# intel/neural-speed

Measured on NVIDIA H100. Metric: decode tokens/s + prefill tok/s Llama-2-7B Q4_0 @1 GPU; % HBM roofline, higher is better.
Workload: dtype int8xint4->f32 (q8_0 x q4_0)

## Files before the change

### neural_speed_b200/csrc/abi.cu

```cuda
#include <atomic>
#include <cstdarg>
#include <cstring>
#include <mutex>
#include <unordered_map>
#include <vector>

#include "nsb.cuh"
#include "btla_planes.h"

static thread_local char g_err[512] = "";
static std::atomic<unsigned long long> g_launches{0};

void ns_set_error(const char* fmt, ...) {
  va_list ap;
  va_start(ap, fmt);
  vsnprintf(g_err, sizeof(g_err), fmt, ap);
  va_end(ap);
}
[[noreturn]] void ns_fatal(const char* fmt, ...) {
  va_list ap;
  va_start(ap, fmt);
  fprintf(stderr, "Err: ");
  vfprintf(stderr, fmt, ap);
  fprintf(stderr, "\n");
// ... 753 lines not shown
  if (!ids || ids_stride < 1 || id < 0 || id >= ids_stride || n_as < 1 || n_as > 256 || m < 1) {
    ns_set_error("ns_mul_mat_id: invalid ids (stride=%d id=%d n_as=%d m=%d)", ids_stride, id, n_as, m);
    return NS_E_INVALID;
  }
  std::vector<int32_t> host;
  const int32_t* h = ids;
  if (ids_on_device) {
    host.resize((size_t)m * ids_stride);
    NS_CUDA_TRY(cudaMemcpyAsync(host.data(), ids, host.size() * sizeof(int32_t), cudaMemcpyDeviceToHost, st));
    NS_CUDA_TRY(cudaStreamSynchronize(st));
    h = host.data();
  }
  std::vector<int> count((size_t)n_as, 0);
  for (int t = 0; t < m; ++t) {
    const int e = h[(size_t)t * ids_stride + id];
    if (e < 0 || e >= n_as) {
      ns_set_error("ns_mul_mat_id: expert id %d of token %d outside [0, %d)", e, t, n_as);
      return NS_E_INVALID;
    }
    ++count[(size_t)e];
  }
  pl->span.assign((size_t)n_as, {0, 0});
  int at = 0;
  for (int e = 0; e < n_as; ++e) {
    pl->span[(size_t)e] = {at, at};
    at += count[(size_t)e];
  }
  pl->order.assign((size_t)m, 0);
  for (int t = 0; t < m; ++t) pl->order[(size_t)pl->span[(size_t)h[(size_t)t * ids_stride + id]].second++] = t;
  pl->identity = true;
  for (int t = 0; t < m; ++t) pl->identity = pl->identity && pl->order[(size_t)t] == t;
  return NS_OK;
}

extern "C" int ns_moe_plan(const int32_t* ids, int ids_stride, int id, int m, int n_as, int* order, int* span) {
  ExpertPlan pl;
  if (int rc = plan_experts(ids, ids_stride, id, 0, m, n_as, nullptr, &pl)) return rc;
  if (order) memcpy(order, pl.order.data(), (size_t)m * sizeof(int));
  if (span)
    for (int e = 0; e < n_as; ++e) {
      span[2 * e] = pl.span[(size_t)e].first;
      span[2 * e + 1] = pl.span[(size_t)e].second;
    }
  return pl.identity ? 1 : 0;
}

struct ExpertScratch {
  int* order;
  float *xg, *yg;
  void* ws;
};
static int expert_scratch(const ExpertPlan& pl, int m, int k, int n, size_t mm_ws, cudaStream_t st, ExpertScratch* sc) {
  const size_t ob = ns_round_up((size_t)m * 4, 256), xb = ns_round_up((size_t)m * k * 4, 256), yb = ns_round_up((size_t)m * n * 4, 256);
  char* base = (char*)scratch_get(st, ob + xb + yb + mm_ws + 256);
  if (!base) return NS_E_CUDA;
  sc->order = (int*)base;
  sc->xg = (float*)(base + ob);
  sc->yg = (float*)(base + ob + xb);
  sc->ws = base + ob + xb + yb;
  if (!pl.identity) NS_CUDA_TRY(cudaMemcpyAsync(sc->order, pl.order.data(), (size_t)m * 4, cudaMemcpyHostToDevice, st));
  return NS_OK;
}

extern "C" int ns_mul_mat_id(const ns_weight* const* experts, int n_as, const int32_t* ids, int ids_stride, int id, int ids_on_device,
                             const float* act, int lda, float* dst, int ldo, int m, int flags, void* queue) {
  if (int rc = ns_ensure_device()) return rc;
  if (!experts || !act || !dst || n_as < 1 || m < 1) return NS_E_INVALID;
  for (int e = 0; e < n_as; ++e)
    if (!experts[e] || experts[e]->n != experts[0]->n || experts[e]->k != experts[0]->k) {
      ns_set_error("ns_mul_mat_id: expert %d missing or of another shape", e);
      return NS_E_INVALID;
    }
  const int n = experts[0]->n, k = experts[0]->k;
  if (lda < k || ldo < n) return NS_E_INVALID;
  cudaStream_t st = stream_of(queue);
  ExpertPlan pl;
  if (int rc = plan_experts(ids, ids_stride, id, ids_on_device, m, n_as, st, &pl)) return rc;
  ExpertScratch sc;
  if (int rc = expert_scratch(pl, m, k, n, ns_device_workspace_bytes(m, k), st, &sc)) return rc;
  const float* x = act;
  float* y = dst;
  int ldx = lda, ldy = ldo;
  if (!pl.identity) {
    if (int rc = ns_launch_move_rows(true, act, lda, sc.order, sc.xg, k, m, k, st)) return rc;
    x = sc.xg, y = sc.yg, ldx = k, ldy = n;
  }
  for (int e = 0; e < n_as; ++e) {
    const int b = pl.span[(size_t)e].first, c = pl.span[(size_t)e].second - b;
    if (c == 0) continue;
    if (int rc = mul_mat_impl(experts[e], x + (size_t)b * ldx, ldx, y + (size_t)b * ldy, ldy, c, nullptr, nullptr, flags, sc.ws, (void*)st,
                              nullptr, 0.f))
      return rc;
  }
  if (!pl.identity) return ns_launch_move_rows(false, sc.yg, n, sc.order, dst, ldo, m, n, st);
  return NS_OK;
}

extern "C" int ns_ffn_id(const ns_weight* const* gate, const ns_weight* const* down, const ns_weight* const* up, int n_as, int gelu,
                         const int32_t* ids, int ids_stride, int id, int ids_on_device, const float* act, int lda, float* tmp,
                         float* dst, int ldo, int m, void* queue) {
  if (int rc = ns_ensure_device()) return rc;
  if (!gate || !down || !up || !act || !tmp || !dst || n_as < 1 || m < 1) return NS_E_INVALID;
  for (int e = 0; e < n_as; ++e)
    if (!gate[e] || !down[e] || !up[e] || gate[e]->n != gate[0]->n || gate[e]->k != gate[0]->k || down[e]->n != down[0]->n ||
        down[e]->k != gate[0]->n || up[e]->n != gate[0]->n || up[e]->k != gate[0]->k) {
      ns_set_error("ns_ffn_id: expert %d missing or of another shape", e);
      return NS_E_INVALID;
    }
  const int k = gate[0]->k, fmid = gate[0]->n, n = down[0]->n;
  if (lda < k || ldo < n) return NS_E_INVALID;
  cudaStream_t st = stream_of(queue);
  ExpertPlan pl;
  if (int rc = plan_experts(ids, ids_stride, id, ids_on_device, m, n_as, st, &pl)) return rc;
  ExpertScratch sc;
  if (int rc = expert_scratch(pl, m, k, n, ns_device_workspace_bytes(m, k > fmid ? k : fmid), st, &sc)) return rc;
  const float* x = act;
  float* y = dst;
  int ldx = lda, ldy = ldo;
  if (!pl.identity) {
    if (int rc = ns_launch_move_rows(true, act, lda, sc.order, sc.xg, k, m, k, st)) return rc;
    x = sc.xg, y = sc.yg, ldx = k, ldy = n;
  }
  for (int e = 0; e < n_as; ++e) {
    const int b = pl.span[(size_t)e].first, c = pl.span[(size_t)e].second - b;
    if (c == 0) continue;
    if (int rc = ffn_impl(gate[e], down[e], up[e], gelu ? NS_ELT_GELU : NS_ELT_DEFAULT, nullptr, nullptr, 0, x + (size_t)b * ldx, ldx,
                          tmp + (size_t)2 * b * fmid, y + (size_t)b * ldy, ldy, c, sc.ws, (void*)st))
      return rc;
  }
  if (!pl.identity) return ns_launch_move_rows(false, sc.yg, n, sc.order, dst, ldo, m, n, st);
  return NS_OK;
}

extern "C" int ns_prepare_activation(const ns_weight* w, const float* act, int lda, int m, void* workspace, void* queue) {
  if (int rc = ns_ensure_device()) return rc;
  if (!w || !act || !workspace || m < 1 || m > ns_gemv_tile_rows(w) || lda < w->k) {
    ns_set_error("ns_prepare_activation: invalid arguments (m=%d)", m);
    return NS_E_INVALID;
  }
  return ns_launch_act_prep(act, lda, m, w, workspace, stream_of(queue));
}

extern "C" int ns_matmul_prepared(const ns_weight* const* weights, int nw, int mode, const void* workspace, float* dst,
                                  int ldo, int m, const float* bias, int bias_bcast, const float* residual, float* aux,
                                  void* queue) {
  if (int rc = ns_ensure_device()) return rc;
  if (!weights || nw < 1 || nw > 3 || mode < 0 || mode > 2 || !workspace || !dst) {
    ns_set_error("ns_matmul_prepared: invalid arguments");
    return NS_E_INVALID;
  }
  return ns_launch_gemv(weights, nw, mode, workspace, dst, ldo, m, m, bias, bias_bcast, residual, aux, stream_of(queue));
}

struct ns_graph {
  cudaGraph_t graph;
  cudaGraphExec_t exec;
};
extern "C" int ns_graph_begin(void* queue) {
  if (int rc = ns_ensure_device()) return rc;
  NS_CUDA_TRY(cudaStreamBeginCapture(stream_of(queue), cudaStreamCaptureModeThreadLocal));
  return NS_OK;
}
extern "C" ns_graph* ns_graph_end(void* queue) {
  cudaGraph_t g = nullptr;
  if (!ns_cuda_ok(cudaStreamEndCapture(stream_of(queue), &g), "cudaStreamEndCapture") || !g) return nullptr;
  cudaGraphExec_t e = nullptr;
  if (!ns_cuda_ok(cudaGraphInstantiate(&e, g, 0), "cudaGraphInstantiate")) {
    cudaGraphDestroy(g);
    return nullptr;
  }
  ns_graph* r = new ns_graph();
  r->graph = g;
  r->exec = e;
  return r;
}
extern "C" int ns_graph_launch(ns_graph* g, void* queue) {
  if (!g) return NS_E_INVALID;
  NS_CUDA_TRY(cudaGraphLaunch(g->exec, stream_of(queue)));
  return NS_OK;
}
extern "C" void ns_graph_free(ns_graph* g) {
  if (!g) return;
  cudaGraphExecDestroy(g->exec);
  cudaGraphDestroy(g->graph);
  delete g;
}

extern "C" void bestla_init(void) { (void)ns_ensure_device(); }
extern "C" int bestla_set_threads(int nth) { return nth; }
extern "C" void* bestla_get_thread_handle(void) { return nullptr; }
extern "C" void bestla_timer(bool) {}

extern "C" void* bestla_create_device(bool profile) {
  if (ns_ensure_device()) ns_fatal("bestla_create_device: %s", g_err);
  ns_device* d = new ns_device();
  d->dev = g_default.dev;
  d->profile = profile;
  if (cudaStreamCreateWithFlags(&d->stream, cudaStreamNonBlocking) != cudaSuccess) ns_fatal("cudaStreamCreate failed");
  return d;
}
extern "C" void* bestla_get_device_queue(void* device) { return device ? (void*)((ns_device*)device)->stream : nullptr; }
extern "C" void bestla_release_device(void* device) {
  if (!device) return;
  ns_device* d = (ns_device*)device;
  cudaStreamSynchronize(d->stream);
  {
    std::lock_guard<std::mutex> lk(g_mu);
    auto it = g_scratch.find(d->stream);
    if (it != g_scratch.end()) {
      cudaFree(it->second.p);
      g_scratch.erase(it);
    }
  }
  cudaStreamDestroy(d->stream);
  delete d;
}
extern "C" size_t bestla_device_gmem_size(void* device) {
  (void)device;
  if (ns_ensure_device()) return 0;
  size_t fr = 0, tot = 0;
  cudaMemGetInfo(&fr, &tot);
  return tot;
}
extern "C" void* bestla_device_malloc(size_t size, void* queue) {
  (void)queue;
  if (ns_ensure_device()) ns_fatal("bestla_device_malloc: %s", g_err);
  void* p = nullptr;
  if (cudaMalloc(&p, size) != cudaSuccess) return nullptr;
  return p;
}
extern "C" void bestla_device_free(void* ptr, void* queue) {
  if (!ptr) return;
  cudaStreamSynchronize(stream_of(queue));
  cudaFree(ptr);
}
extern "C" void bestla_device_memcpy(void* dstptr, const void* srcptr, size_t size, void* queue) {
  if (ns_ensure_device()) ns_fatal("bestla_device_memcpy: %s", g_err);
  if (cudaMemcpyAsync(dstptr, srcptr, size, cudaMemcpyDefault, stream_of(queue)) != cudaSuccess)
    ns_fatal("bestla_device_memcpy failed: %s", cudaGetErrorString(cudaGetLastError()));
}
extern "C" void bestla_device_memcpy_sync(void* dstptr, const void* srcptr, size_t size, void* queue) {
  bestla_device_memcpy(dstptr, srcptr, size, queue);
  cudaStreamSynchronize(stream_of(queue));
}
extern "C" void bestla_device_sync(void* queue) {
  if (ns_ensure_device()) ns_fatal("bestla_device_sync: %s", g_err);
  if (cudaStreamSynchronize(stream_of(queue)) != cudaSuccess)
    ns_fatal("bestla_device_sync: %s", cudaGetErrorString(cudaGetLastError()));
}
extern "C" size_t bestla_device_storage_size(void) { return sizeof(ns_weight); }
extern "C" size_t ns_device_storage_bytes(const void* hoststor) {
  BlobView v;
  ns_weight w;
  if (!parse_blob(hoststor, &v) || blob_to_weight_meta(v, &w)) return 0;
  return weight_image_bytes(&w, v.shuffle != nullptr);
}
extern "C" void bestla_device_load_storage(void* hoststor, void* devstor, void* deviceptr, void* queue) {
  if (ns_ensure_device()) ns_fatal("bestla_device_load_storage: %s", g_err);
  BlobView v;
  ns_weight* w = (ns_weight*)devstor;
  if (!devstor || !deviceptr || !parse_blob(hoststor, &v) || blob_to_weight_meta(v, w))
    ns_fatal("bestla_device_load_storage: invalid parameters (%s)", g_err);
  w->base = deviceptr;
  w->external = 1;
  w->total_bytes = weight_image_bytes(w, v.shuffle != nullptr);
  weight_carve(w, deviceptr, v.shuffle != nullptr);
  if (cudaMemsetAsync(deviceptr, 0, w->total_bytes, stream_of(queue)) != cudaSuccess) ns_fatal("cudaMemset failed");
  if (blob_upload_repack(v, w, stream_of(queue))) ns_fatal("bestla_device_load_storage: %s", g_err);
}
extern "C" void bestla_device_f32f32_forward(float* activation, void* weiptr, float* output, int m, int n, int k, int lda,
                                             int ldo, void* workspace, void* queue) {
  const ns_weight* w = (const ns_weight*)weiptr;
  if (!w || w->n != n || w->k != k) ns_fatal("invalid parameters");
  (void)lda;
  if (ns_mul_mat(w, activation, k, output, ldo, m, nullptr, nullptr, 0, workspace, queue))
    ns_fatal("bestla_device_f32f32_forward: %s", g_err);
}

struct CacheEntry {
  ns_weight* w;
  size_t tag;
};
static std::unordered_map<const void*, CacheEntry> g_cache;

static size_t blob_tag(const void* blob, size_t nbytes) {
  size_t t = 1469598103934665603ull;
  const unsigned char* p = (const unsigned char*)blob;
  const size_t head = nbytes < 64 ? nbytes : 64;
  for (size_t i = 0; i < head; ++i) t = (t ^ p[i]) * 1099511628211ull;
  if (nbytes > 72) {
    const size_t span = nbytes - 8, steps = 256;
    for (size_t j = 0; j < steps; ++j) {
      const size_t off = 64 + (size_t)((__uint128_t)(span - 64) * j / steps);
      unsigned long long v;
      memcpy(&v, p + off, 8);
      t = (t ^ (size_t)v) * 1099511628211ull;
    }
  }
  return (t ^ nbytes) * 1099511628211ull;
}
static size_t btla_blob_bytes(const void* blob) {
  size_t msize = 0;
  memcpy(&msize, blob, sizeof(size_t));
  return (msize >= 64 && msize <= ((size_t)1 << 40)) ? msize : 64;
}

// ... 315 lines not shown
```

### neural_speed_b200/csrc/gemv_ring_impl.cuh

```cuda
#pragma once
#include "act_quant.cuh"

namespace {

constexpr int kConsumers = 7;
constexpr int kThreads = (kConsumers + 1) * 32;

__device__ __forceinline__ uint32_t smem_u32(const void* p) { return (uint32_t)__cvta_generic_to_shared(p); }
__device__ __forceinline__ void mbar_init(uint32_t bar, int count) {
  asm volatile("mbarrier.init.shared::cta.b64 [%0], %1;" ::"r"(bar), "r"(count) : "memory");
}
__device__ __forceinline__ void mbar_expect_tx(uint32_t bar, uint32_t bytes) {
  asm volatile("mbarrier.arrive.expect_tx.shared::cta.b64 _, [%0], %1;" ::"r"(bar), "r"(bytes) : "memory");
}
__device__ __forceinline__ void mbar_arrive(uint32_t bar) {
  asm volatile("mbarrier.arrive.shared::cta.b64 _, [%0];" ::"r"(bar) : "memory");
}
__device__ __forceinline__ void mbar_wait(uint32_t bar, uint32_t parity) {
  uint32_t ok;
  do {
    asm volatile(
        "{\n"
        ".reg .pred p;\n"
        "mbarrier.try_wait.parity.shared::cta.b64 p, [%1], %2;\n"
        "selp.u32 %0, 1, 0, p;\n"
        "}\n"
        : "=r"(ok)
        : "r"(bar), "r"(parity)
        : "memory");
  } while (!ok);
}
__device__ __forceinline__ void bulk_g2s(uint32_t dst, const void* src, uint32_t bytes, uint32_t bar) {
  asm volatile("cp.async.bulk.shared::cluster.global.mbarrier::complete_tx::bytes [%0], [%1], %2, [%3];" ::"r"(dst), "l"(src),
               "r"(bytes), "r"(bar)
               : "memory");
}
__device__ __forceinline__ uint4 lds128(uint32_t a) {
  uint4 r;
  asm volatile("ld.shared.v4.u32 {%0,%1,%2,%3}, [%4];" : "=r"(r.x), "=r"(r.y), "=r"(r.z), "=r"(r.w) : "r"(a));
  return r;
}
__device__ __forceinline__ uint2 lds64(uint32_t a) {
  uint2 r;
  asm volatile("ld.shared.v2.u32 {%0,%1}, [%2];" : "=r"(r.x), "=r"(r.y) : "r"(a));
  return r;
}
__device__ __forceinline__ uint32_t lds32(uint32_t a) {
  uint32_t r;
  asm volatile("ld.shared.u32 %0, [%1];" : "=r"(r) : "r"(a));
  return r;
}
__device__ __forceinline__ uint32_t lds16(uint32_t a) {
  unsigned short r;
  asm volatile("ld.shared.u16 %0, [%1];" : "=h"(r) : "r"(a));
  return r;
}
__device__ __forceinline__ int lds8s(uint32_t a) {
  int r;
  asm volatile("ld.shared.s8 %0, [%1];" : "=r"(r) : "r"(a));
  return r;
}
template <int STYPE>
__device__ __forceinline__ float lds_scale(uint32_t base, int idx) {
  if (STYPE == NS_S_F32) return __uint_as_float(lds32(base + 4 * idx));
  if (STYPE == NS_S_F16) return __half2float(__ushort_as_half((unsigned short)lds16(base + 2 * idx)));
  return __uint_as_float(lds16(base + 2 * idx) << 16);
}

struct QuantIn {
  const float* in;
  const float* norm_w;
  float eps;
  int lda, k, kpad, group;
  int act_row, meta_off, meta_stride;
};

__device__ __forceinline__ void sts64(uint32_t a, uint32_t x, uint32_t y) {
  asm volatile("st.shared.v2.u32 [%0], {%1,%2};" ::"r"(a), "r"(x), "r"(y) : "memory");
}
__device__ __forceinline__ float4 ldcg4(const float* p) {
  float4 r;
  asm volatile("ld.global.cg.v4.f32 {%0,%1,%2,%3}, [%4];" : "=f"(r.x), "=f"(r.y), "=f"(r.z), "=f"(r.w) : "l"(p));
  return r;
}
__device__ __forceinline__ float ldcg1(const float* p) {
  float r;
  asm volatile("ld.global.cg.f32 %0, [%1];" : "=f"(r) : "l"(p));
  return r;
}
template <int BAR, int NT>
__device__ __forceinline__ void bar_sync() {
  asm volatile("bar.sync %0, %1;" ::"n"(BAR), "n"(NT) : "memory");
}

template <int NT>
__device__ __forceinline__ void prefetch_norm_w(const float* __restrict__ norm_w, int k, int kpad, int tid, float (&gw)[3][8]) {
  const int ngroups8 = kpad >> 3;
#pragma unroll
  for (int it = 0; it < 3; ++it) {
    const int e = it * NT + tid, k0 = e * 8;
    if (e < ngroups8 && k0 + 8 <= k) {
      const float4 w0 = __ldg(reinterpret_cast<const float4*>(norm_w + k0)), w1 = __ldg(reinterpret_cast<const float4*>(norm_w + k0 + 4));
      gw[it][0] = w0.x; gw[it][1] = w0.y; gw[it][2] = w0.z; gw[it][3] = w0.w;
      gw[it][4] = w1.x; gw[it][5] = w1.y; gw[it][6] = w1.z; gw[it][7] = w1.w;
    } else {
#pragma unroll
      for (int i = 0; i < 8; ++i) gw[it][i] = (e < ngroups8 && k0 + i < k) ? __ldg(norm_w + k0 + i) : 0.f;
    }
  }
}

template <int NI, int NT>
__device__ __forceinline__ void load_passes(const float* row, int eb, int tid, int ngroups8, int k, float (&vv)[NI][8]) {
#pragma unroll
  for (int it = 0; it < NI; ++it) {
    const int e = eb + it * NT + tid;
    const int k0 = e * 8;
    if (e < ngroups8 && k0 + 8 <= k) {
      const float4 x0 = ldcg4(row + k0), x1 = ldcg4(row + k0 + 4);
      vv[it][0] = x0.x; vv[it][1] = x0.y; vv[it][2] = x0.z; vv[it][3] = x0.w;
      vv[it][4] = x1.x; vv[it][5] = x1.y; vv[it][6] = x1.z; vv[it][7] = x1.w;
    } else {
#pragma unroll
      for (int i = 0; i < 8; ++i) vv[it][i] = (e < ngroups8 && k0 + i < k) ? ldcg1(row + k0 + i) : 0.f;
    }
  }
}

template <int COMP, int NT, bool NORM>
__device__ __forceinline__ void quantise_to_smem(const QuantIn& P, int M, uint32_t smem_base, float* red, const float (*gw)[8]) {
  constexpr int NI = 3;
  const int tpb = (COMP == NS_COMP_Q8_0 ? 32 : P.group) >> 3;
  const int ngroups8 = P.kpad >> 3;
  const int tid = threadIdx.x;
  const bool single = ngroups8 <= NI * NT;
  const bool norm = NORM && P.norm_w != nullptr;
  for (int m = 0; m < M; ++m) {
    const float* row = P.in + (size_t)m * P.lda;
    const uint32_t img = smem_base + (uint32_t)m * P.act_row;
    const uint32_t meta = smem_base + P.meta_off + 8u * (uint32_t)(m * P.meta_stride);
    float vv[NI][8];
    auto sum_sq = [&](float ss) {
#pragma unroll
      for (int it = 0; it < NI; ++it)
#pragma unroll
        for (int i = 0; i < 8; ++i) ss = fmaf(vv[it][i], vv[it][i], ss);
      return ss;
    };
    if (NORM && single) load_passes<NI, NT>(row, 0, tid, ngroups8, P.k, vv);
    float inv = 1.f;
    if (norm) {
      float ss = 0.f;
      if (single) {
        ss = sum_sq(ss);
      } else {
        for (int eb = 0; eb < ngroups8; eb += NI * NT) {
          load_passes<NI, NT>(row, eb, tid, ngroups8, P.k, vv);
          ss = sum_sq(ss);
        }
      }
      ss = warp_sum(ss);
      bar_sync<1, NT>();
      if ((tid & 31) == 0) red[tid >> 5] = ss;
      bar_sync<1, NT>();
      float tot = 0.f;
#pragma unroll
      for (int i = 0; i < NT / 32; ++i) tot += red[i];
      inv = 1.f / sqrtf(tot / (float)P.k + P.eps);
    }
    for (int eb = 0; eb < ngroups8; eb += NI * NT) {
      if (!(NORM && single)) load_passes<NI, NT>(row, eb, tid, ngroups8, P.k, vv);
#pragma unroll
      for (int it = 0; it < NI; ++it) {
        const int e0 = eb + it * NT;
        if (e0 >= ngroups8) break;
        const int e = e0 + tid;
        const bool live = e < ngroups8;
        const int k0 = e * 8;
        float v[8];
#pragma unroll
        for (int i = 0; i < 8; ++i) v[i] = vv[it][i];
        if (norm && gw != nullptr && single) {
#pragma unroll
          for (int i = 0; i < 8; ++i) v[i] = v[i] * inv * gw[it][i];
        } else if (norm) {
          if (live && k0 + 8 <= P.k) {
            const float4 w0 = __ldg((const float4*)(P.norm_w + k0)), w1 = __ldg((const float4*)(P.norm_w + k0 + 4));
            v[0] = v[0] * inv * w0.x; v[1] = v[1] * inv * w0.y; v[2] = v[2] * inv * w0.z; v[3] = v[3] * inv * w0.w;
            v[4] = v[4] * inv * w1.x; v[5] = v[5] * inv * w1.y; v[6] = v[6] * inv * w1.z; v[7] = v[7] * inv * w1.w;
          } else {
#pragma unroll
            for (int i = 0; i < 8; ++i) v[i] = (live && k0 + i < P.k) ? v[i] * inv * __ldg(P.norm_w + k0 + i) : 0.f;
          }
        }
        float vmax = nsq::range_start<COMP>((k0 | (tpb * 8 - 1)) >= P.k), vmin = 0.f;
#pragma unroll
        for (int i = 0; i < 8; ++i) nsq::range_fold<COMP>(v[i], vmax, vmin);
        nsq::range_reduce<COMP>(vmax, vmin, tpb);
        const nsq::BlockQuant bq = nsq::block_quant<COMP>(vmax, vmin);
        int q[8], sa = 0;
#pragma unroll
        for (int i = 0; i < 8; ++i) {
          q[i] = k0 + i < P.k ? nsq::quant_code<COMP>(v[i], bq) : bq.za;
          sa += q[i];
        }
        sa += __shfl_xor_sync(0xffffffffu, sa, 1);
        sa += __shfl_xor_sync(0xffffffffu, sa, 2);
        if (live) {
          uint32_t w[2] = {0u, 0u};
#pragma unroll
          for (int i = 0; i < 8; ++i) w[nsq::dp4a_pos(i) >> 2] |= (uint32_t)(q[i] & 0xff) << (8 * (nsq::dp4a_pos(i) & 3));
          const int c = e >> 2, i = e & 3;
          sts64(img + nsq::ring_offset((uint32_t)c, (uint32_t)i * 8u), w[0], w[1]);
          if (i == 0) {
            const int2 mw = nsq::meta_word(bq.scale, sa, bq.za);
            sts64(meta + 8u * (uint32_t)c, (uint32_t)mw.x, (uint32_t)mw.y);
          }
        }
      }
    }
  }
}

struct PairSrc {
  const uint8_t* r0;
  const uint8_t* r1;
  long long out0, out1;
  bool valid1;
};

__device__ __forceinline__ PairSrc resolve_pair(const GemvParams& P, int p) {
  PairSrc s;
  if (P.mode == NS_GEMV_GATE_UP_SILU) {
    s.r0 = P.rows[0] + (size_t)p * P.pitch;
    s.r1 = P.rows[1] + (size_t)p * P.pitch;
    s.out0 = s.out1 = p;
    s.valid1 = true;
    return s;
  }
  int row = 2 * p, wi = 0;
  if (P.nw > 1 && row >= P.n[0]) {
    row -= P.n[0];
    wi = 1;
    if (P.nw > 2 && row >= P.n[1]) {
      row -= P.n[1];
      wi = 2;
    }
  }
  s.valid1 = row + 1 < P.n[wi];
  s.r0 = P.rows[wi] + (size_t)row * P.pitch;
  s.r1 = s.valid1 ? s.r0 + P.pitch : s.r0;
  s.out0 = P.dst_off[wi] + row;
  s.out1 = s.out0 + 1;
  return s;
}

struct RingCfg {
  int ring_off;
  int stages;
  int units;
  int active;
  int act_row;
  int red_off;
  uint32_t cpg_magic;
};

__device__ __forceinline__ PairSrc resolve_single(const GemvParams& P, int u) {
  PairSrc s;
  int row = u, wi = 0;
  if (P.nw > 1 && row >= P.n[0]) {
    row -= P.n[0];
    wi = 1;
    if (P.nw > 2 && row >= P.n[1]) {
      row -= P.n[1];
      wi = 2;
    }
  }
  s.r0 = s.r1 = P.rows[wi] + (size_t)row * P.pitch;
  s.out0 = s.out1 = P.dst_off[wi] + row;
  s.valid1 = false;
  return s;
}

template <int AMODE, int M, bool ASYM, int STYPE, int ROWS, bool NORM, int NC>
__global__ void __launch_bounds__((NC + (NC > kConsumers ? 2 : 1)) * 32, NC > kConsumers ? 1 : 2)
    gemv_ring_kernel(const GemvParams P, const RingCfg R) {
  constexpr int NP = NC > kConsumers ? 2 : 1;
  extern __shared__ __align__(128) unsigned char smem[];
  const int lane = threadIdx.x & 31, warp = threadIdx.x >> 5;
  const int stage_bytes = ROWS * P.pitch;
  const int stages = R.stages;
  const uint32_t smem_base = smem_u32(smem);
  const uint32_t ring = smem_base + R.ring_off;
  const uint32_t full0 = ring + (uint32_t)stages * stage_bytes;
  const uint32_t empty0 = full0 + 8u * stages;

  pdl_launch_dependents();
  if (threadIdx.x == 0) {
    for (int s = 0; s < stages; ++s) {
      mbar_init(full0 + 8 * s, 1);
      mbar_init(empty0 + 8 * s, 1);
    }
    asm volatile("fence.mbarrier_init.release.cluster;" ::: "memory");
  }
  __syncthreads();

  const int first = blockIdx.x;
  const int gstride = (int)gridDim.x;
  const int my_units = first < R.units ? (R.units - first + gstride - 1) / gstride : 0;

  if (warp >= NC) {
    if (lane == 0) {
      int s = warp - NC;
      uint32_t phase = 0;
      for (int j = warp - NC; j < my_units; j += NP) {
        if (j >= stages) mbar_wait(empty0 + 8 * s, phase ^ 1);
        const PairSrc ps = ROWS == 2 ? resolve_pair(P, first + j * gstride) : resolve_single(P, first + j * gstride);
        const uint32_t dst = ring + (uint32_t)s * stage_bytes;
        mbar_expect_tx(full0 + 8 * s, (uint32_t)stage_bytes);
        bulk_g2s(dst, ps.r0, (uint32_t)P.pitch, full0 + 8 * s);
        if (ROWS == 2) bulk_g2s(dst + P.pitch, ps.r1, (uint32_t)P.pitch, full0 + 8 * s);
        s += NP;
        if (s >= stages) {
          s -= stages;
          phase ^= 1;
        }
      }
    }
    return;
  }

  float gw[NORM ? 3 : 1][8];
  bool gw_pref = false;
  if constexpr (NORM) {
    gw_pref = P.norm_w != nullptr && (P.kpad >> 3) <= 3 * NC * 32;
    if (gw_pref) prefetch_norm_w<NC * 32>(P.norm_w, P.k, P.kpad, (int)threadIdx.x, gw);
  }
  pdl_wait();
  if (P.act_f32) {
    const QuantIn qi{P.act_f32, NORM ? P.norm_w : nullptr, P.norm_eps, P.lda, P.k, P.kpad, P.comp == NS_COMP_Q8_0 ? 32 : P.group,
                     R.act_row, P.meta_off, P.meta_stride};
    float* red = reinterpret_cast<float*>(smem + R.red_off);
    const float(*gwp)[8] = gw_pref ? gw : nullptr;
    if (AMODE == A_U8) quantise_to_smem<NS_COMP_INT8, NC * 32, NORM>(qi, P.m, smem_base, red, gwp);
    else if (P.comp == NS_COMP_Q8_0) quantise_to_smem<NS_COMP_Q8_0, NC * 32, NORM>(qi, P.m, smem_base, red, gwp);
    else quantise_to_smem<NS_COMP_INT8_S8, NC * 32, NORM>(qi, P.m, smem_base, red, gwp);
  } else {
    const uint4* src = reinterpret_cast<const uint4*>(P.act);
    uint4* dstv = reinterpret_cast<uint4*>(smem);
    const int nvec = P.act_bytes >> 4;
    for (int i = threadIdx.x; i < nvec; i += NC * 32) dstv[i] = src[i];
  }
  asm volatile("bar.sync 1, %0;" ::"n"(NC * 32) : "memory");
  const uint32_t meta_s = smem_base + P.meta_off;
  const int nchunks = P.kpad >> 5;

  int s = warp;
  uint32_t phase = 0;

  const int active = R.active;
  if (warp >= active) return;
  for (int j = warp; j < my_units; j += active) {
    const PairSrc ps = ROWS == 2 ? resolve_pair(P, first + j * gstride) : resolve_single(P, first + j * gstride);
    mbar_wait(full0 + 8 * s, phase);
    const uint32_t r0 = ring + (uint32_t)s * stage_bytes;
    const uint32_t r1 = ROWS == 2 ? r0 + P.pitch : r0;
    const uint32_t rb[2] = {r0, r1};

    float acc[ROWS][M];
#pragma unroll
    for (int r = 0; r < ROWS; ++r)
#pragma unroll
      for (int m = 0; m < M; ++m) acc[r][m] = 0.f;

#pragma unroll 2
    for (int c = lane; c < nchunks; c += 32) {
      const int gi = (P.cpg == 1) ? c : (int)__umulhi((uint32_t)c, R.cpg_magic);
      uint4 wv[ROWS];
      float ws[ROWS];
      int off[ROWS];
#pragma unroll
      for (int r = 0; r < ROWS; ++r) {
        wv[r] = lds128(rb[r] + 16 * c);
        ws[r] = lds_scale<STYPE>(rb[r] + P.sc_off, gi);
        off[r] = 8;
        if (ASYM) off[r] += lds8s(rb[r] + P.zp_off + gi);
      }
      uint32_t lo[ROWS][4], hi[ROWS][4];
      int su[ROWS];
#pragma unroll
      for (int r = 0; r < ROWS; ++r) {
        su[r] = 0;
        const uint32_t ww[4] = {wv[r].x, wv[r].y, wv[r].z, wv[r].w};
#pragma unroll
        for (int i = 0; i < 4; ++i) {
          lo[r][i] = ww[i] & 0x0F0F0F0Fu;
          hi[r][i] = ww[i] & 0xF0F0F0F0u;
        }
        if (AMODE == A_U8) {
          int sl = 0, sh = 0;
#pragma unroll
          for (int i = 0; i < 4; ++i) {
            sl = dp4a_uu(lo[r][i], 0x01010101u, sl);
            sh = dp4a_uu(hi[r][i], 0x01010101u, sh);
          }
          su[r] = sl + (sh >> 4);
        }
      }
      const uint32_t a_off = (uint32_t)(c >> 5) * 1024u + (uint32_t)(c & 31) * 16u;
#pragma unroll
      for (int m = 0; m < M; ++m) {
        const uint32_t ab = smem_base + (uint32_t)m * R.act_row + a_off;
        const uint4 a0 = lds128(ab), a1 = lds128(ab + 512);
        const uint2 mt = lds64(meta_s + 8u * (uint32_t)(m * P.meta_stride + c));
        const float a_scale = __uint_as_float(mt.x);
        const int sa = (int)(short)(mt.y & 0xffff);
#pragma unroll
        for (int r = 0; r < ROWS; ++r) {
          int pl = 0, ph = 0;
          if (AMODE == A_U8) {
            pl = dp4a_uu(a0.x, lo[r][0], pl); ph = dp4a_uu(a0.y, hi[r][0], ph);
            pl = dp4a_uu(a0.z, lo[r][1], pl); ph = dp4a_uu(a0.w, hi[r][1], ph);
            pl = dp4a_uu(a1.x, lo[r][2], pl); ph = dp4a_uu(a1.y, hi[r][2], ph);
            pl = dp4a_uu(a1.z, lo[r][3], pl); ph = dp4a_uu(a1.w, hi[r][3], ph);
          } else {
            pl = dp4a_us(lo[r][0], (int)a0.x, pl); ph = dp4a_us(hi[r][0], (int)a0.y, ph);
            pl = dp4a_us(lo[r][1], (int)a0.z, pl); ph = dp4a_us(hi[r][1], (int)a0.w, ph);
            pl = dp4a_us(lo[r][2], (int)a1.x, pl); ph = dp4a_us(hi[r][2], (int)a1.y, ph);
            pl = dp4a_us(lo[r][3], (int)a1.z, pl); ph = dp4a_us(hi[r][3], (int)a1.w, ph);
          }
          int isum = pl + (ph >> 4) - off[r] * sa;
          if (AMODE == A_U8) {
            const int za = (int)((mt.y >> 16) & 0xff);
            isum -= za * (su[r] - 32 * off[r]);
          }
          acc[r][m] = fmaf((float)isum, a_scale * ws[r], acc[r][m]);
        }
      }
    }
    __syncwarp();
    if (lane == 0) mbar_arrive(empty0 + 8 * s);
    s += active;
    if (s >= stages) {
      s -= stages;
      phase ^= 1u;
    }

#pragma unroll
    for (int r = 0; r < ROWS; ++r)
#pragma unroll
      for (int m = 0; m < M; ++m) acc[r][m] = warp_sum(acc[r][m]);
    if (lane == 0) {
      if (ROWS == 2 && P.mode == NS_GEMV_GATE_UP_SILU) {
#pragma unroll
        for (int m = 0; m < M; ++m) {
          if (m < P.m) {
            const float g = acc[0][m], up = acc[ROWS - 1][m];
            const float sg = P.eltop == NS_ELT_GELU ? ns_gelu(g) : ns_silu(g);
            if (P.aux) P.aux[(size_t)m * P.ldo + ps.out0] = sg;
            P.dst[(size_t)m * P.ldo + ps.out0] = sg * up;
          }
        }
      } else {
#pragma unroll
        for (int r = 0; r < ROWS; ++r) {
          if (r == 1 && !ps.valid1) continue;
          const long long out = r ? ps.out1 : ps.out0;
#pragma unroll
          for (int m = 0; m < M; ++m) {
            if (m < P.m) {
              const size_t o = (size_t)m * P.ldo + out;
              float v = acc[r][m];
              if (P.bias) v += P.bias_bcast ? P.bias[out] : P.bias[o];
              if (P.eltop == NS_ELT_GELU) v = ns_gelu(v);
              if (P.residual) v += P.residual[o];
              P.dst[o] = v;
            }
          }
        }
      }
    }
  }
}

struct RingPlan {
  int rows, stages, active, ctas;
  size_t budget;
  double score;
};

static RingPlan plan_ring(const GemvParams& P, size_t act_region, bool wide) {
  static const int env_budget = getenv("NS_RING_BUDGET_KB") ? atoi(getenv("NS_RING_BUDGET_KB")) : 0;
  static const int env_rows = getenv("NS_RING_ROWS") ? atoi(getenv("NS_RING_ROWS")) : 0;
  const size_t budgets[2] = {(size_t)(env_budget > 0 ? env_budget : 113) * 1024, 200 * 1024};
  RingPlan best = {0, 0, 0, 0, 0, -1.0};
  for (int rows = 2; rows >= 1; --rows) {
    if (rows == 1 && P.mode == NS_GEMV_GATE_UP_SILU) continue;
    if (env_rows && rows != env_rows && !(env_rows == 1 && P.mode == NS_GEMV_GATE_UP_SILU)) continue;
    const int stage_bytes = rows * P.pitch;
    for (int i = 0; i < 2; ++i) {
      if (wide && i == 0) continue;
      const int kc = (wide && i == 1) ? 2 * kConsumers : kConsumers;
      int raw = 0;
      if (budgets[i] > act_region + 64) raw = (int)((budgets[i] - act_region - 64) / (stage_bytes + 16));
      if (raw > (wide ? 56 : 32)) raw = wide ? 56 : 32;
      const int ac = raw < kc ? raw : kc;
      if (ac < 1) continue;
      const int st = raw - raw % ac;
      const int ctas = i == 0 ? 2 : 1;
      const double score = ctas * ac * (rows == 2 ? 1.1 : 1.0) + 0.001 * st;
      if (score > best.score) best = RingPlan{rows, st, ac, ctas, budgets[i], score};
    }
  }
  return best;
}

template <int AMODE, int M, bool ASYM, int STYPE, int ROWS, bool NORM, int NC = kConsumers>
int launch_rows(const GemvParams& P, const RingPlan& plan, size_t act_region, int act_row, int red_off, cudaStream_t st) {
  auto kern = gemv_ring_kernel<AMODE, M, ASYM, STYPE, ROWS, NORM, NC>;
  constexpr int threads = (NC + (NC > kConsumers ? 2 : 1)) * 32;
  static bool attr_set = false;
  if (!attr_set) {
    NS_CUDA_TRY(cudaFuncSetAttribute(kern, cudaFuncAttributeMaxDynamicSharedMemorySize, 200 * 1024));
    attr_set = true;
  }
  const int stage_bytes = ROWS * P.pitch;
  const size_t smem = act_region + (size_t)plan.stages * stage_bytes + (size_t)plan.stages * 16;
  static const int env_cps = getenv("NS_RING_CPS") ? atoi(getenv("NS_RING_CPS")) : 0;
  const int ctas_per_sm = plan.ctas == 1 ? 1 : (env_cps > 0 ? env_cps : 2);
  RingCfg R;
  R.ring_off = (int)act_region;
  R.stages = plan.stages;
  R.active = plan.active;
  R.act_row = act_row;
  R.red_off = red_off;
  if (ROWS == 2) {
    R.units = P.npairs;
  } else {
    long long rows = 0;
    for (int i = 0; i < P.nw; ++i) rows += P.n[i];
    R.units = (int)rows;
  }
  R.cpg_magic = P.cpg > 1 ? (uint32_t)((0x100000000ull + (uint64_t)P.cpg - 1) / (uint64_t)P.cpg) : 0u;
  int grid = ns_num_sms() * ctas_per_sm;
  if (grid > R.units) grid = R.units;
  if (grid < 1) grid = 1;
  static const bool dbg = getenv("NS_RING_DEBUG") != nullptr;
  if (dbg)
    fprintf(stderr, "gemv_ring: k=%d pitch=%d rows/stage=%d stages=%d active=%d smem=%zu ctas/sm=%d\n", P.k, P.pitch, ROWS, plan.stages,
            plan.active, smem, ctas_per_sm);
  NS_CUDA_TRY(ns_launch_pdl(kern, dim3(grid), dim3(threads), smem, st, P, R));
  ns_count_launch();
  return NS_OK;
}

}
```

### neural_speed_b200/csrc/nsb.cuh

```cuda
#pragma once
#include <cuda_bf16.h>
#include <cuda_fp16.h>
#include <cuda_runtime.h>
#include <stdint.h>
#include <stdio.h>
#include <stdlib.h>

#include "../../include/ns_b200.h"

struct ns_weight {
  int n, k, kpad;
  int group, ngroups;
  int wfmt, stype, comp, asym;
  uint8_t* rows;
  int pitch, q_bytes, sc_off, zp_off;
  int* shuffle;
  void* base;
  size_t total_bytes;
  int external;
  int f4kind;
};
enum { NS_F4_NF4 = 0, NS_F4_BNB = 1, NS_F4_E2M1 = 2 };

static inline size_t ns_round_up(size_t a, size_t b) { return (a + b - 1) / b * b; }
static inline int ns_stype_size(int stype) { return stype == NS_S_F32 ? 4 : 2; }

static inline void ns_weight_layout(ns_weight* w) {
  w->kpad = (int)ns_round_up((size_t)w->k, 32);
  if (w->group <= 0 || w->group > w->k) w->group = w->k;
  w->ngroups = (w->k + w->group - 1) / w->group;
  w->q_bytes = (w->wfmt == NS_W_S8) ? w->kpad : w->kpad / 2;
  w->sc_off = w->q_bytes;
  w->zp_off = (int)ns_round_up((size_t)w->sc_off + (size_t)w->ngroups * ns_stype_size(w->stype), 16);
  w->pitch = (int)ns_round_up((size_t)w->zp_off + (w->asym ? w->ngroups : 0), 16);
}

void ns_set_error(const char* fmt, ...);
[[noreturn]] void ns_fatal(const char* fmt, ...);
bool ns_cuda_ok(cudaError_t e, const char* what);
int ns_ensure_device();
void ns_count_launch(int n = 1);
int ns_num_sms();
cudaStream_t ns_stream_of(void* queue);

#define NS_CUDA_TRY(expr)                             \
  do {                                                \
    if (!ns_cuda_ok((expr), #expr)) return NS_E_CUDA; \
  } while (0)

size_t ns_act_workspace_bytes(int m, int kpad);
static inline int ns_meta_stride(int kpad) { return (int)ns_round_up((size_t)(kpad >> 5), 2); }

int ns_launch_act_prep(const float* act, int lda, int m, const ns_weight* w, void* ws, cudaStream_t st);
int ns_gemv_tile_rows(const ns_weight* w);
int ns_launch_gemv(const ns_weight* const* ws_, int nw, int mode, const void* act_ws, float* dst, int ldo, int m,
                   int m_total, const float* bias, int bias_bcast, const float* residual, float* aux, cudaStream_t st,
                   const float* act_f32 = nullptr, int lda = 0, int eltop = 0, const float* norm_w = nullptr, float norm_eps = 0.f,
                   int one_image = 0);
bool ns_gemv_fused_quant_ok(const ns_weight* w);
int ns_gemv_check(const ns_weight* const* ws, int nw, int mode);
int ns_launch_repack_q4_0(const void* rows_dev, size_t nb01, ns_weight* w, cudaStream_t st);
int ns_launch_repack_canonical(const int8_t* q_kn_dev, const float* sc_dev, const int8_t* zp_dev, ns_weight* w,
                               cudaStream_t st);
int ns_launch_repack_btla(const void* qbuf_dev, const void* sc_dev, int src_stype, const int8_t* zp_dev, int cstep,
                          int kpad_src, int ntile, int packrow, int is_float, ns_weight* w, cudaStream_t st);
int ns_launch_dequant(const ns_weight* w, float* dst, int ld, cudaStream_t st);
int ns_launch_random_weight(ns_weight* w, unsigned seed, cudaStream_t st);

void ns_q6k_layout(ns_weight* w);
int ns_launch_repack_q6k(const void* rows_dev, size_t nb01, ns_weight* w, cudaStream_t st);
size_t ns_q6k_workspace_bytes(int m, int k);
int ns_launch_dequant_q6k(const ns_weight* w, float* dst, int ld, cudaStream_t st);
int ns_launch_mul_mat_q6k(const ns_weight* w, const float* act, int lda, float* dst, int ldo, int m, const float* bias,
                          int bias_bcast, const float* residual, void* ws, cudaStream_t st);

enum { NS_PATH_GEMV, NS_PATH_IMMA, NS_PATH_TC, NS_PATH_Q6K };
enum { NS_NODE_PLAIN, NS_NODE_QKV, NS_NODE_FFN };
int ns_route(int kind, const ns_weight* const* w, int m, int flags);
int ns_ffn_silu_residual(const ns_weight* w1, const ns_weight* w2, const ns_weight* w3, const float* act, int lda, float* tmp,
                         float* dst, int ldo, int m, const float* residual, void* workspace, cudaStream_t st,
                         const float* norm_w = nullptr, float norm_eps = 0.f, int one_image = 0);
int ns_mul_mat_engine(const ns_weight* w, const float* act, int lda, float* dst, int ldo, int m, const float* residual, void* workspace,
                      cudaStream_t st, const float* norm_w, float norm_eps);
int ns_mul_qkv_norm(const ns_weight* wq, const ns_weight* wk, const ns_weight* wv, const float* act, int lda, float* dst, int ldo,
                    int m, void* workspace, void* queue, const float* norm_w, float norm_eps);

int ns_launch_move_rows(bool gather, const float* src, int ld_src, const int* idx_dev, float* dst, int ld_dst, int rows, int cols,
                        cudaStream_t st);

size_t ns_gemm_tc_workspace_bytes(int m, int kpad);
bool ns_gemm_tc_supported(const ns_weight* w);
int ns_launch_act_bf16(const ns_weight* w, const float* act, int lda, int m, void* ws, cudaStream_t st);
int ns_launch_gemm_tc(const ns_weight* w, const void* ws, float* dst, int ldo, int m, const float* bias, int bias_bcast,
                      const float* residual, cudaStream_t st);
int ns_launch_silu_mul(const float* g, const float* u, float* out, float* aux, size_t total, cudaStream_t st, int eltop = 0);
int ns_launch_gelu(float* x, size_t total, cudaStream_t st);
bool ns_launch_silu_mul_bf16(const ns_weight* w2, const float* g, const float* u, int m, void* ws, cudaStream_t st, int eltop, int* rc);

bool ns_gemm_imma_supported(const ns_weight* const* ws, int nw, int m);
size_t ns_gemm_imma_workspace_bound(int m, int kpad);
int ns_launch_gemm_imma(const ns_weight* const* ws, int nw, int mode, const float* act, int lda, float* dst, int ldo, int m,
                        const float* bias, int bias_bcast, const float* residual, int eltop, void* workspace, cudaStream_t st);

enum { NS_GEMV_PLAIN = 0, NS_GEMV_CONCAT = 1, NS_GEMV_GATE_UP_SILU = 2 };
enum { NS_ELT_DEFAULT = 0, NS_ELT_GELU = 1 };
enum { A_S8 = 0, A_U8 = 1, A_F32 = 2 };

struct GemvParams {
  const uint8_t* rows[3];
  int n[3];
  long long dst_off[3];
  int nw, mode;
  int k, kpad, group, ngroups, stype;
  int cpg;
  int pitch, q_bytes, sc_off, zp_off;
  const void* act;
  const float* act_f32;
  int lda, comp;
  int act_bytes;
  int meta_off;
  int meta_stride;
  float* dst;
  int ldo, m;
  const float* bias;
  int bias_bcast;
  const float* residual;
  float* aux;
  int npairs;
  int eltop;
  int f4kind;
  const float* norm_w;
  float norm_eps;
  int one_image;
};
int ns_launch_gemv_ring(const GemvParams& P, int amode, bool asym, int mt, cudaStream_t st);
int ns_launch_gemv_ring_wide(const GemvParams& P, int amode, bool asym, size_t act_region, int act_row, int red_off, cudaStream_t st,
                             bool* taken);

template <typename... Args>
static inline cudaError_t ns_launch_pdl(void (*kern)(Args...), dim3 grid, dim3 block, size_t smem, cudaStream_t st,
                                        Args... args) {
  cudaLaunchConfig_t cfg = {};
  cfg.gridDim = grid;
  cfg.blockDim = block;
  cfg.dynamicSmemBytes = smem;
  cfg.stream = st;
  cudaLaunchAttribute attr[1];
  attr[0].id = cudaLaunchAttributeProgrammaticStreamSerialization;
  attr[0].val.programmaticStreamSerializationAllowed = 1;
  static const bool no_pdl = getenv("NS_NO_PDL") != nullptr;
  cfg.attrs = attr;
  cfg.numAttrs = no_pdl ? 0 : 1;
  return cudaLaunchKernelEx(&cfg, kern, args...);
}

#ifdef __CUDACC__
__device__ __forceinline__ uint4 ld_nc_v4(const void* p) {
  uint4 r;
  asm volatile("ld.global.nc.L1::no_allocate.v4.u32 {%0,%1,%2,%3}, [%4];"
               : "=r"(r.x), "=r"(r.y), "=r"(r.z), "=r"(r.w)
               : "l"(p));
  return r;
}
__device__ __forceinline__ float ns_gelu(float x) {
  return 0.5f * x * (1.f + tanhf(0.7978845834732056f * (x + 0.044714998453855515f * x * x * x)));
}
__device__ __forceinline__ float ns_silu(float x) { return x / (1.f + expf(-x)); }
__device__ __forceinline__ void pdl_wait() { asm volatile("griddepcontrol.wait;" ::: "memory"); }
__device__ __forceinline__ void pdl_launch_dependents() { asm volatile("griddepcontrol.launch_dependents;" ::: "memory"); }

__device__ __forceinline__ float ns_scale_at(const void* s, int stype, int idx) {
  if (stype == NS_S_F32) return reinterpret_cast<const float*>(s)[idx];
  if (stype == NS_S_F16) return __half2float(__ushort_as_half(reinterpret_cast<const unsigned short*>(s)[idx]));
  return __uint_as_float(static_cast<uint32_t>(reinterpret_cast<const unsigned short*>(s)[idx]) << 16);
}
__device__ __forceinline__ float warp_sum(float v) {
#pragma unroll
  for (int o = 16; o > 0; o >>= 1) v += __shfl_xor_sync(0xffffffffu, v, o);
  return v;
}
__device__ __forceinline__ int dp4a_uu(unsigned a, unsigned b, int c) {
  int d;
  asm("dp4a.u32.u32 %0, %1, %2, %3;" : "=r"(d) : "r"(a), "r"(b), "r"(c));
  return d;
}
__device__ __forceinline__ int dp4a_ss(int a, int b, int c) {
  int d;
  asm("dp4a.s32.s32 %0, %1, %2, %3;" : "=r"(d) : "r"(a), "r"(b), "r"(c));
  return d;
}
__device__ __forceinline__ int dp4a_us(unsigned a, int b, int c) {
  int d;
  asm("dp4a.u32.s32 %0, %1, %2, %3;" : "=r"(d) : "r"(a), "r"(b), "r"(c));
  return d;
}
static __device__ __constant__ const float NS_F4_LUT[3][16] = {
    {0.f, -0.6961928009986877f, -0.5250730514526367f, -0.39491748809814453f, -0.28444138169288635f, -0.18477343022823334f, -0.09105003625154495f, -1.f, 0.07958029955625534f, 0.16093020141124725f, 0.24611230194568634f, 0.33791524171829224f, 0.44070982933044434f, 0.5626170039176941f, 0.7229568362236023f, 1.0f},
    {0.f, 5.208333333e-03f, 0.66666667f, 1.f, 0.33333333f, 0.5f, 0.16666667f, 0.25f,
     -0.f, -5.208333333e-03f, -0.66666667f, -1.f, -0.33333333f, -0.5f, -0.16666667f, -0.25f},
    {0.f, 0.010416666666666666f, 0.16666666666666666f, 0.25f, 0.3333333333333333f, 0.5f, 0.6666666666666666f, 1.f,
     -0.f, -0.010416666666666666f, -0.16666666666666666f, -0.25f, -0.3333333333333333f, -0.5f, -0.6666666666666666f, -1.f}};
#endif
```

Measured before the change: 653.8.

## Prefetch next ring GEMV's weights into L2 during graph capture and evict-first loads

Result: faster. 675.5 (median of 6 runs) (+3.3%).

```diff
diff --git a/neural_speed_b200/csrc/abi.cu b/neural_speed_b200/csrc/abi.cu
--- a/neural_speed_b200/csrc/abi.cu
+++ b/neural_speed_b200/csrc/abi.cu
@@ -929,6 +929,75 @@
   return ns_launch_gemv(weights, nw, mode, workspace, dst, ldo, m, m, bias, bias_bcast, residual, aux, stream_of(queue));
 }
 
+constexpr int kRingPrefetchBytes = 32 * 1024;
+
+struct RingNodeRec {
+  unsigned long long capture_id;
+  cudaGraphNode_t node;
+  void (*kern)(GemvParams, RingCfg);
+  dim3 grid, block;
+  size_t smem;
+  GemvParams P;
+  RingCfg R;
+};
+static std::mutex g_ring_mu;
+static std::unordered_map<cudaStream_t, RingNodeRec> g_ring_last;
+
+int ns_ring_launch(void (*kern)(GemvParams, RingCfg), dim3 grid, dim3 block, size_t smem, cudaStream_t st, const GemvParams& P,
+                   const RingCfg& R, int stage_rows) {
+  NS_CUDA_TRY(ns_launch_pdl(kern, grid, block, smem, st, P, R));
+  cudaStreamCaptureStatus cs = cudaStreamCaptureStatusNone;
+  unsigned long long id = 0;
+  const cudaGraphNode_t* deps = nullptr;
+  size_t ndeps = 0;
+  NS_CUDA_TRY(cudaStreamGetCaptureInfo_v3(st, &cs, &id, nullptr, &deps, nullptr, &ndeps));
+  std::lock_guard<std::mutex> lk(g_ring_mu);
+  if (cs != cudaStreamCaptureStatusActive) {
+    g_ring_last.erase(st);
+    return NS_OK;
+  }
+  auto it = g_ring_last.find(st);
+  if (it != g_ring_last.end() && it->second.capture_id == id) {
+    RingNodeRec& prev = it->second;
+    GemvNext& N = prev.P.next;
+    for (int i = 0; i < 3; ++i) {
+      N.rows[i] = P.rows[i];
+      N.n[i] = P.n[i];
+    }
+    N.nw = P.nw;
+    N.mode = P.mode;
+    N.pitch = P.pitch;
+    N.stage_rows = stage_rows;
+    N.units = R.units;
+    N.grid = (int)grid.x;
+    N.budget = kRingPrefetchBytes;
+    void* args[2] = {&prev.P, &prev.R};
+    cudaKernelNodeParams kp = {};
+    kp.func = (void*)prev.kern;
+    kp.gridDim = prev.grid;
+    kp.blockDim = prev.block;
+    kp.sharedMemBytes = (unsigned)prev.smem;
+    kp.kernelParams = args;
+    NS_CUDA_TRY(cudaGraphKernelNodeSetParams(prev.node, &kp));
+  }
+  cudaGraphNodeType type = cudaGraphNodeTypeEmpty;
+  if (ndeps == 1) NS_CUDA_TRY(cudaGraphNodeGetType(deps[0], &type));
+  if (type != cudaGraphNodeTypeKernel) {
+    g_ring_last.erase(st);
+    return NS_OK;
+  }
+  RingNodeRec& rec = g_ring_last[st];
+  rec.capture_id = id;
+  rec.node = deps[0];
+  rec.kern = kern;
+  rec.grid = grid;
+  rec.block = block;
+  rec.smem = smem;
+  rec.P = P;
+  rec.R = R;
+  return NS_OK;
+}
+
 struct ns_graph {
   cudaGraph_t graph;
   cudaGraphExec_t exec;
diff --git a/neural_speed_b200/csrc/gemv_ring_impl.cuh b/neural_speed_b200/csrc/gemv_ring_impl.cuh
--- a/neural_speed_b200/csrc/gemv_ring_impl.cuh
+++ b/neural_speed_b200/csrc/gemv_ring_impl.cuh
@@ -30,10 +30,18 @@
         : "memory");
   } while (!ok);
 }
-__device__ __forceinline__ void bulk_g2s(uint32_t dst, const void* src, uint32_t bytes, uint32_t bar) {
-  asm volatile("cp.async.bulk.shared::cluster.global.mbarrier::complete_tx::bytes [%0], [%1], %2, [%3];" ::"r"(dst), "l"(src),
-               "r"(bytes), "r"(bar)
+__device__ __forceinline__ uint64_t l2_evict_first() {
+  uint64_t pol;
+  asm volatile("createpolicy.fractional.L2::evict_first.b64 %0, 1.0;" : "=l"(pol));
+  return pol;
+}
+__device__ __forceinline__ void bulk_g2s(uint32_t dst, const void* src, uint32_t bytes, uint32_t bar, uint64_t pol) {
+  asm volatile("cp.async.bulk.shared::cluster.global.mbarrier::complete_tx::bytes.L2::cache_hint [%0], [%1], %2, [%3], %4;" ::"r"(dst),
+               "l"(src), "r"(bytes), "r"(bar), "l"(pol)
                : "memory");
+}
+__device__ __forceinline__ void bulk_prefetch_l2(const void* src, uint32_t bytes) {
+  asm volatile("cp.async.bulk.prefetch.L2.global [%0], %1;" ::"l"(src), "r"(bytes) : "memory");
 }
 __device__ __forceinline__ uint4 lds128(uint32_t a) {
   uint4 r;
@@ -229,7 +237,11 @@
   bool valid1;
 };
 
-__device__ __forceinline__ PairSrc resolve_pair(const GemvParams& P, int p) {
+__device__ __forceinline__ long long dst_base(const GemvParams& P, int wi) { return P.dst_off[wi]; }
+__device__ __forceinline__ long long dst_base(const GemvNext&, int) { return 0; }
+
+template <class PP>
+__device__ __forceinline__ PairSrc resolve_pair(const PP& P, int p) {
   PairSrc s;
   if (P.mode == NS_GEMV_GATE_UP_SILU) {
     s.r0 = P.rows[0] + (size_t)p * P.pitch;
@@ -250,22 +262,13 @@
   s.valid1 = row + 1 < P.n[wi];
   s.r0 = P.rows[wi] + (size_t)row * P.pitch;
   s.r1 = s.valid1 ? s.r0 + P.pitch : s.r0;
-  s.out0 = P.dst_off[wi] + row;
+  s.out0 = dst_base(P, wi) + row;
   s.out1 = s.out0 + 1;
   return s;
 }
 
-struct RingCfg {
-  int ring_off;
-  int stages;
-  int units;
-  int active;
-  int act_row;
-  int red_off;
-  uint32_t cpg_magic;
-};
-
-__device__ __forceinline__ PairSrc resolve_single(const GemvParams& P, int u) {
+template <class PP>
+__device__ __forceinline__ PairSrc resolve_single(const PP& P, int u) {
   PairSrc s;
   int row = u, wi = 0;
   if (P.nw > 1 && row >= P.n[0]) {
@@ -277,7 +280,7 @@
     }
   }
   s.r0 = s.r1 = P.rows[wi] + (size_t)row * P.pitch;
-  s.out0 = s.out1 = P.dst_off[wi] + row;
+  s.out0 = s.out1 = dst_base(P, wi) + row;
   s.valid1 = false;
   return s;
 }
@@ -313,17 +316,36 @@
     if (lane == 0) {
       int s = warp - NC;
       uint32_t phase = 0;
+      const uint64_t pol = l2_evict_first();
       for (int j = warp - NC; j < my_units; j += NP) {
         if (j >= stages) mbar_wait(empty0 + 8 * s, phase ^ 1);
         const PairSrc ps = ROWS == 2 ? resolve_pair(P, first + j * gstride) : resolve_single(P, first + j * gstride);
         const uint32_t dst = ring + (uint32_t)s * stage_bytes;
         mbar_expect_tx(full0 + 8 * s, (uint32_t)stage_bytes);
-        bulk_g2s(dst, ps.r0, (uint32_t)P.pitch, full0 + 8 * s);
-        if (ROWS == 2) bulk_g2s(dst + P.pitch, ps.r1, (uint32_t)P.pitch, full0 + 8 * s);
+        bulk_g2s(dst, ps.r0, (uint32_t)P.pitch, full0 + 8 * s, pol);
+        if (ROWS == 2) bulk_g2s(dst + P.pitch, ps.r1, (uint32_t)P.pitch, full0 + 8 * s, pol);
         s += NP;
         if (s >= stages) {
           s -= stages;
           phase ^= 1;
+        }
+      }
+      const GemvNext& N = P.next;
+      if (first < N.units) {
+        const int nstage = N.stage_rows * N.pitch;
+        int nmine = (N.units - first + N.grid - 1) / N.grid;
+        if (nmine > N.budget / nstage) nmine = N.budget / nstage;
+        const int pw = warp - NC;
+        const int j0 = my_units - stages;
+        int j = j0 < pw ? pw : j0 + ((pw - j0) % NP + NP) % NP;
+        int jn = pw, credit = 0;
+        for (; j < my_units && jn < nmine; j += NP) {
+          mbar_wait(full0 + 8 * (j % stages), (uint32_t)(j / stages) & 1u);
+          for (credit += stage_bytes; jn < nmine && credit >= nstage; jn += NP, credit -= nstage) {
+            const PairSrc ps = N.stage_rows == 2 ? resolve_pair(N, first + jn * N.grid) : resolve_single(N, first + jn * N.grid);
+            bulk_prefetch_l2(ps.r0, (uint32_t)N.pitch);
+            if (ps.valid1) bulk_prefetch_l2(ps.r1, (uint32_t)N.pitch);
+          }
         }
       }
     }
@@ -549,7 +571,7 @@
   if (dbg)
     fprintf(stderr, "gemv_ring: k=%d pitch=%d rows/stage=%d stages=%d active=%d smem=%zu ctas/sm=%d\n", P.k, P.pitch, ROWS, plan.stages,
             plan.active, smem, ctas_per_sm);
-  NS_CUDA_TRY(ns_launch_pdl(kern, dim3(grid), dim3(threads), smem, st, P, R));
+  if (int rc = ns_ring_launch(kern, dim3(grid), dim3(threads), smem, st, P, R, ROWS)) return rc;
   ns_count_launch();
   return NS_OK;
 }
diff --git a/neural_speed_b200/csrc/nsb.cuh b/neural_speed_b200/csrc/nsb.cuh
--- a/neural_speed_b200/csrc/nsb.cuh
+++ b/neural_speed_b200/csrc/nsb.cuh
@@ -105,6 +105,15 @@
 enum { NS_GEMV_PLAIN = 0, NS_GEMV_CONCAT = 1, NS_GEMV_GATE_UP_SILU = 2 };
 enum { NS_ELT_DEFAULT = 0, NS_ELT_GELU = 1 };
 enum { A_S8 = 0, A_U8 = 1, A_F32 = 2 };
+
+struct GemvNext {
+  const uint8_t* rows[3];
+  int n[3];
+  int nw, mode, pitch;
+  int stage_rows;
+  int units, grid;
+  int budget;
+};
 
 struct GemvParams {
   const uint8_t* rows[3];
@@ -132,7 +141,20 @@
   const float* norm_w;
   float norm_eps;
   int one_image;
-};
+  GemvNext next;
+};
+
+struct RingCfg {
+  int ring_off;
+  int stages;
+  int units;
+  int active;
+  int act_row;
+  int red_off;
+  uint32_t cpg_magic;
+};
+int ns_ring_launch(void (*kern)(GemvParams, RingCfg), dim3 grid, dim3 block, size_t smem, cudaStream_t st, const GemvParams& P,
+                   const RingCfg& R, int stage_rows);
 int ns_launch_gemv_ring(const GemvParams& P, int amode, bool asym, int mt, cudaStream_t st);
 int ns_launch_gemv_ring_wide(const GemvParams& P, int amode, bool asym, size_t act_region, int act_row, int red_off, cudaStream_t st,
                              bool* taken);
diff --git a/profiles/ring_boundary.py b/profiles/ring_boundary.py
--- /dev/null
+++ b/profiles/ring_boundary.py
@@ -0,0 +1,107 @@
+import argparse
+import ctypes as C
+import os
+import subprocess
+import sys
+
+sys.path.insert(0, os.path.dirname(os.path.dirname(os.path.abspath(__file__))))
+import numpy as np
+import torch
+
+import neural_speed_b200 as ns
+
+SHAPES = [(4096, 4096, 8), (11008, 4096, 3), (4096, 11008, 3)]
+
+
+def card():
+    try:
+        return subprocess.run(["nvidia-smi", "--query-gpu=name,power.limit,clocks.max.sm", "--format=csv,noheader"],
+                              capture_output=True, text=True, timeout=30).stdout.strip().splitlines()[0]
+    except Exception as e:
+        return f"{torch.cuda.get_device_name(0)}, power limit and clock unknown ({e})"
+
+
+def main():
+    ap = argparse.ArgumentParser()
+    ap.add_argument("--repeats", type=int, default=15, help="alternations of (a) and (b) per shape")
+    ap.add_argument("--replays", type=int, default=20, help="graph replays per timed window")
+    args = ap.parse_args()
+    assert torch.cuda.is_available(), "needs the GPU"
+    L = ns.lib()
+    L.bestla_init()
+    queue = L.bestla_get_device_queue(L.bestla_create_device(False))
+    stream = torch.cuda.ExternalStream(queue)
+    torch.manual_seed(1234)
+    cp = lambda t: C.c_void_p(t.data_ptr())
+
+    def q4_0(n, k):
+        w = torch.randn(n, k, device="cuda") * 0.02
+        rows = torch.empty(n * (k // 32) * 18, dtype=torch.uint8, device="cuda")
+        torch.cuda.synchronize()
+        assert L.ns_device_quantize_q4_0(cp(w), cp(rows), n, k, queue) == 0, ns.last_error()
+        h = ns.Weight.from_q4_0_device(rows.data_ptr(), n, k, k // 32 * 18, queue)
+        L.bestla_device_sync(queue)
+        return h
+
+    def capture(fn):
+        assert L.ns_graph_begin(queue) == 0, ns.last_error()
+        fn()
+        g = L.ns_graph_end(queue)
+        assert g, ns.last_error()
+        return C.c_void_p(g)
+
+    def timed(g):
+        e0, e1 = torch.cuda.Event(enable_timing=True), torch.cuda.Event(enable_timing=True)
+        e0.record(stream)
+        for _ in range(args.replays):
+            L.ns_graph_launch(g, queue)
+        e1.record(stream)
+        e1.synchronize()
+        return e0.elapsed_time(e1) * 1e3 / args.replays
+
+    print(f"card: {card()}")
+    print(f"{args.repeats} alternations of (a) and (b) per shape, {args.replays} replays per timed window, CUDA events")
+    for n, k, nsets in SHAPES:
+        sets = [[q4_0(n, k) for _ in range(3)] for _ in range(nsets)]
+        x = torch.randn(1, k, device="cuda")
+        dst = torch.zeros(3, 1, n, device="cuda")
+        ws = torch.zeros(L.ns_device_workspace_bytes(4, max(n, k)), dtype=torch.uint8, device="cuda")
+        torch.cuda.synchronize()
+
+        def fused():
+            for s in sets:
+                assert L.ns_mul_qkv(s[0].h, s[1].h, s[2].h, cp(x), k, cp(dst), n, 1, cp(ws), queue) == 0, ns.last_error()
+
+        def split():
+            for s in sets:
+                for i in range(3):
+                    assert L.ns_mul_mat(s[i].h, cp(x), k, C.c_void_p(dst.data_ptr() + i * n * 4), n, 1, None, None, 0, cp(ws),
+                                        queue) == 0, ns.last_error()
+
+        fused()
+        split()
+        L.bestla_device_sync(queue)
+        ga, gb = capture(fused), capture(split)
+        for _ in range(3):
+            timed(ga)
+            timed(gb)
+        ta, tb = [], []
+        for _ in range(args.repeats):
+            ta.append(timed(ga))
+            tb.append(timed(gb))
+        ta, tb = np.array(ta), np.array(tb)
+        per = (tb - ta) / (nsets * 2)
+        nbytes = 3 * nsets * n * (k // 32) * 18
+        print(f"3 x {n}x{k} Q4_0, {nsets} sets ({nbytes / 1e6:.0f} MB per replay): (a) {nsets} launches median {np.median(ta):.1f} us "
+              f"({nbytes / np.median(ta) / 1e3:.0f} GB/s), (b) {3 * nsets} launches median {np.median(tb):.1f} us "
+              f"({nbytes / np.median(tb) / 1e3:.0f} GB/s)")
+        print(f"  per boundary: median {np.median(per):.3f} us, min {per.min():.3f}, max {per.max():.3f} "
+              f"(128 boundaries: {128 * np.median(per):.1f} us)")
+        L.ns_graph_free(ga)
+        L.ns_graph_free(gb)
+        del sets, x, dst, ws
+        torch.cuda.empty_cache()
+
+
+if __name__ == "__main__":
+    main()
```
